# Critical-Infrastructure-Systems-Lab/ldsr

Hardware: AMD Instinct MI355X
Metric: restart x EM-iteration / s (T=1000, p=1, q=2) (higher is better)
Workload: dtype f64; 1 GPU; cfg2: synthetic T=1000 p=1 q=2, 1 series x 4096 restarts/GPU, niter=100, tol=0, dense mask; cells_rank0=4096, cells_total=4096, niter=100, algo=3

## Files before the change

include/ldsr_hip.h:

```cpp
#ifndef LDSR_HIP_H
#define LDSR_HIP_H

#include <stddef.h>

#ifdef __cplusplus
extern "C" {
#endif

#define LDSR_OK 0
#define LDSR_EINVAL 1
#define LDSR_EUNSUPPORTED 2
#define LDSR_EHIP 3
#define LDSR_EINTERRUPTED 4
#define LDSR_EINTERNAL 5

#define LDSR_CELL_OK 0
#define LDSR_CELL_NONFINITE 1
#define LDSR_CELL_SINGULAR 2
#define LDSR_CELL_INTERRUPTED 3

#define LDSR_ALGO_AUTO 0
#define LDSR_ALGO_SERIAL 1
#define LDSR_ALGO_SCAN 2
#define LDSR_ALGO_PAIR 3
// ... 29 lines not shown
int ldsr_em_restart_groups(int n_devices, const int *devices, int n_groups, ldsr_group *groups,
                           int niter, double tol, int algo);

int ldsr_em_batch(int device, int n_series, int T, int p, int q, const double *y,
                  const double *u, const double *v, int shared_uv, const int *cell_offsets,
                  const double *theta0, int niter, double tol, int algo,
                  double *theta, double *lik, int *n_iter, int *status, double *liks);

int ldsr_em_batch_multi(int n_devices, const int *devices, int n_series, int T, int p, int q,
                        const double *y, const double *u, const double *v, int shared_uv,
                        const int *cell_offsets, const double *theta0, int niter, double tol,
                        int algo, double *theta, double *lik, int *n_iter, int *status,
                        double *liks);

size_t ldsr_em_workspace_bytes(int n_series, int T, int p, int q, int n_cells, int algo);
int ldsr_em_batch_device(int device, void *stream, int n_series, int T, int p, int q,
                         const double *d_y, const double *d_u, const double *d_v,
                         int shared_uv, const int *cell_offsets, const double *d_theta0,
                         int niter, double tol, int algo, double *d_theta, double *d_lik,
                         int *d_n_iter, int *d_status, double *d_liks, void *d_workspace,
                         size_t workspace_bytes);

int ldsr_em_plan(int T, int p, int q, int niter, double tol, int algo, char *buf, size_t len);

int ldsr_em_batch_device_lead(int device, void *stream, int n_series, int T, int p, int q,
                              const double *d_y, const double *d_u, const double *d_v,
                              int shared_uv, const int *cell_offsets, const double *d_theta0,
                              int niter, double tol, int algo, double *d_theta, double *d_lik,
                              int *d_n_iter, int *d_status, double *d_liks, void *d_workspace,
                              size_t workspace_bytes, int lead_steps);
// ... 107 lines not shown
```

ldsr_amd/_lib.py:

```python
import ctypes as C
import os

_HERE = os.path.dirname(os.path.abspath(__file__))
SO_PATH = os.environ.get("LDSR_HIP_SO") or os.path.join(_HERE, "libldsr_hip.so")

_dp = C.POINTER(C.c_double)
_ip = C.POINTER(C.c_int)
_vp = C.c_void_p

SIGNATURES = {
    "ldsr_last_error": (C.c_char_p, []),
    "ldsr_version": (C.c_char_p, []),
    "ldsr_source_hash": (C.c_char_p, []),
    "ldsr_device_count": (C.c_int, []),
    "ldsr_shutdown": (None, []),
    "ldsr_em_batch": (C.c_int, [C.c_int, C.c_int, C.c_int, C.c_int, C.c_int, _dp, _dp, _dp,
                                C.c_int, _ip, _dp, C.c_int, C.c_double, C.c_int, _dp, _dp, _ip,
                                _ip, _dp]),
    "ldsr_em_batch_multi": (C.c_int, [C.c_int, _ip, C.c_int, C.c_int, C.c_int, C.c_int, _dp, _dp, _dp,
                                      C.c_int, _ip, _dp, C.c_int, C.c_double, C.c_int, _dp, _dp,
                                      _ip, _ip, _dp]),
    "ldsr_em_restart_grid": (C.c_int, [C.c_int, _ip, C.c_int, C.c_int, C.c_int, C.c_int, _dp, _dp, _dp,
                                       C.c_int, _ip, _dp, C.c_int, C.c_double, C.c_int, _dp, _dp,
                                       _ip, _ip, _ip, _dp, _dp, _ip, _dp, _dp, _dp, _dp, _dp]),
    "ldsr_em_restart_groups": (C.c_int, [C.c_int, _ip, C.c_int, _vp, C.c_int, C.c_double, C.c_int]),
    "ldsr_em_plan": (C.c_int, [C.c_int, C.c_int, C.c_int, C.c_int, C.c_double, C.c_int, C.c_char_p,
                               C.c_size_t]),
    "ldsr_em_plan_lead": (C.c_int, [C.c_int, C.c_int, C.c_int, C.c_int, C.c_double, C.c_int, C.c_int,
                                    C.c_char_p, C.c_size_t]),
    "ldsr_em_batch_device_lead": (C.c_int, [C.c_int, _vp, C.c_int, C.c_int, C.c_int, C.c_int, _vp, _vp,
                                            _vp, C.c_int, _ip, _vp, C.c_int, C.c_double, C.c_int, _vp,
                                            _vp, _vp, _vp, _vp, _vp, C.c_size_t, C.c_int]),
    "ldsr_smooth_plan": (C.c_int, [C.c_int, C.c_int, C.c_int, C.c_char_p, C.c_size_t]),
    "ldsr_kernel_inventory": (C.c_size_t, [C.c_char_p, C.c_size_t]),
    "ldsr_last_em_kernel": (C.c_int, [C.c_int, C.c_char_p, C.c_size_t]),
    "ldsr_set_interrupt_callback": (C.c_int, [_vp, _vp]),
    "ldsr_em_workspace_bytes": (C.c_size_t, [C.c_int, C.c_int, C.c_int, C.c_int, C.c_int, C.c_int]),
    "ldsr_em_batch_device": (C.c_int, [C.c_int, _vp, C.c_int, C.c_int, C.c_int, C.c_int, _vp, _vp,
                                       _vp, C.c_int, _ip, _vp, C.c_int, C.c_double, C.c_int, _vp,
                                       _vp, _vp, _vp, _vp, _vp, C.c_size_t]),
    "ldsr_smooth_batch": (C.c_int, [C.c_int, C.c_int, C.c_int, C.c_int, C.c_int, _dp, _dp, _dp,
                                    C.c_int, _ip, _dp, C.c_int, _dp, _dp, _dp, _dp, _dp]),
    "ldsr_mstep_batch": (C.c_int, [C.c_int, C.c_int, C.c_int, C.c_int, C.c_int, _dp, _dp, _dp,
                                   C.c_int, _ip, _dp, _dp, _dp, _dp, _ip]),
    "ldsr_propagate_batch": (C.c_int, [C.c_int, C.c_int, C.c_int, C.c_int, C.c_int, _dp, _dp, _dp,
                                       C.c_int, _ip, _dp, C.c_int, _dp, _dp, _dp, _dp]),
    "ldsr_penalized_lik_batch": (C.c_int, [C.c_int, C.c_int, C.c_int, C.c_int, C.c_int, _dp, _dp, _dp,
                                           C.c_int, _ip, _dp, C.c_double, _dp]),
    "ldsr_ga_batch": (C.c_int, [C.c_int, C.c_int, C.c_int, C.c_int, C.c_int, _dp, _dp, _dp, C.c_int, _dp, _dp,
                                C.c_double, C.c_int, C.c_int, C.c_int, C.c_int, C.c_ulonglong, _dp, C.c_int,
                                _dp, _dp, _ip, _dp, _dp, _dp]),
    "ldsr_ssq_grad_batch": (C.c_int, [C.c_int, C.c_int, C.c_int, C.c_int, C.c_int, _dp, _dp, _dp, C.c_int, _ip,
# ... 92 lines not shown
```

ldsr_amd/csrc/api_em.hip:

```cpp
#include <hip/hip_runtime.h>

#include <algorithm>
#include <cstdio>
#include <cstring>
#include <mutex>
#include <string>
#include <vector>

#include "host_em.h"
#include "em_pair_impl.h"

namespace ldsr_host {

static int device_cu_count(int device) {
    if (device < 0) return 256;
    static std::mutex mu;
    static std::vector<int> cache;
    std::lock_guard<std::mutex> lk(mu);
    if ((int)cache.size() <= device) cache.resize((size_t)device + 1, 0);
    if (!cache[(size_t)device]) {
        int n = 0;
        if (hipDeviceGetAttribute(&n, hipDeviceAttributeMultiprocessorCount, device) != hipSuccess || n <= 0) n = 256;
        cache[(size_t)device] = n;
    }
// ... 1 lines not shown
}

static std::mutex g_last_mu;
static std::vector<std::string> g_last_kernel;
static void remember_kernel(int device, const char *name) {
    std::lock_guard<std::mutex> lk(g_last_mu);
    if ((int)g_last_kernel.size() <= device) g_last_kernel.resize((size_t)device + 1);
    g_last_kernel[(size_t)device] = name;
}
extern "C" int ldsr_last_em_kernel(int device, char *buf, size_t len) {
    std::lock_guard<std::mutex> lk(g_last_mu);
    if (device < 0 || (int)g_last_kernel.size() <= device || g_last_kernel[(size_t)device].empty() || !buf || !len)
        return -1;
    snprintf(buf, len, "%s", g_last_kernel[(size_t)device].c_str());
    return 0;
}

WsLayout ws_layout(int n_series, int T, int PP, int QQ, int shared_uv, int n_cells,
                   int algo, int cpb) {
    WsLayout L;
    size_t o = 0;
    L.sc = o; o = align256(o + sizeof(SeriesConst) * (size_t)n_series);
    L.yp = o; o = align256(o + sizeof(double) * (size_t)n_series * T);
    L.yz = o; o = align256(o + sizeof(double) * (size_t)n_series * T);
    const size_t nuv = shared_uv ? 1 : (size_t)n_series;
    L.up = o; o = align256(o + sizeof(double) * nuv * T * PP);
    L.vp = o; o = align256(o + sizeof(double) * nuv * T * QQ);
    em_scan_layout(T, PP, QQ, &L.img_L, &L.img_NL, &L.img_stride);
    L.img = o; o = align256(o + sizeof(double) * (size_t)L.img_stride * n_series);
    L.img2_stride = 0; L.img3_stride = 0;
    if (PP <= 8 && QQ <= 8 && algo != LDSR_ALGO_SERIAL) {
        L.img2_stride = pair_image_doubles(PP <= 4 && QQ <= 4 ? 32 : 16, PP, QQ, 32);
        L.img3_stride = (long)(T + 32) * PP;
    }
    L.img2 = o; o = align256(o + sizeof(double) * (size_t)L.img2_stride * n_series);
    L.img3 = o; o = align256(o + sizeof(double) * (size_t)L.img3_stride * n_series);
    if (L.img_stride) cpb = std::min(cpb, em_scan_cells_per_block(T, PP, QQ));
    if (PP <= 8 && QQ <= 8 && algo != LDSR_ALGO_SERIAL) cpb = std::min(cpb, 4);
    L.max_blocks = n_cells / cpb + n_series + 1;
    L.blk = o; o = align256(o + sizeof(int) * (3 * (size_t)L.max_blocks + (size_t)n_series + 1));
    L.soc = o; o = align256(o + sizeof(int) * (size_t)(n_cells > 0 ? n_cells : 1));
    L.queue = o; o = align256(o + sizeof(int) * (size_t)n_series);
    const bool may_order = PP <= 4 && QQ <= 4 && algo != LDSR_ALGO_SERIAL;
    L.perm = o; o = align256(o + (may_order ? sizeof(int) * (size_t)(n_cells > 0 ? n_cells : 1) : 0));
    L.perm_key = o; o = align256(o + (may_order ? sizeof(int) * (size_t)(n_cells > 0 ? n_cells : 1) : 0));
    L.scratch_stride = ((long)n_cells + 63) / 64 * 64;
    L.scratch = o;
    if (algo == LDSR_ALGO_SERIAL) o = align256(o + sizeof(double) * 2 * (size_t)T * L.scratch_stride);
    L.total = o;
    return L;
}

extern "C" size_t ldsr_em_workspace_bytes(int n_series, int T, int p, int q, int n_cells,
                                          int algo) {
    if (n_series < 1 || n_cells < 0) return 0;
    EmPlanIn in;
    in.T = T; in.p = p; in.q = q; in.niter = 2; in.algo = algo;
    const EmPlan pl = em_plan(in);
    if (!pl.ok) return 0;
    return ws_layout(n_series, T, pl.PP, pl.QQ, 0, n_cells, pl.algo_layout, pl.layout_cpb).total;
}

extern "C" int ldsr_em_plan_lead(int T, int p, int q, int niter, double tol, int algo, int lead_steps,
                                 char *buf, size_t len) {
    EmPlanIn in;
    in.T = T; in.p = p; in.q = q; in.niter = niter; in.tol = tol; in.algo = algo; in.lead_steps = lead_steps;
    const EmPlan pl = em_plan(in);
    if (!pl.ok) return -1;
    if (buf && len) em_plan_kernel_name(pl, buf, len);
    return pl.algo;
}

extern "C" int ldsr_em_plan(int T, int p, int q, int niter, double tol, int algo, char *buf,
                            size_t len) {
    return ldsr_em_plan_lead(T, p, q, niter, tol, algo, 0, buf, len);
// ... 81 lines not shown
        pp.img2_stride = L.img2_stride;
        pp.L2 = pl.chunk;
        pp.NL2 = pl.lpc;
        pp.lead = pl.lead;
        pp.img3 = (pl.lead > 0 && L.img3_stride) ? (double *)(ws + L.img3) : nullptr;
        pp.img3_stride = L.img3_stride;
    }
    if (pl.steady_order) {
        tab.insert(tab.end(), cell_offsets, cell_offsets + n_series + 1);
        pp.perm = (int *)(ws + L.perm);
        pp.perm_key = (int *)(ws + L.perm_key);
        pp.cell_off = d_tab + 3 * n_blocks;
        pp.theta0 = E.theta0;
        pp.order_cpb = pl.queue ? 0 : cpb;
        pp.order_ntr = pl.chunk - 1;
    }
    rc = stage_h2d_async(E.device, E.stream, d_tab, tab.data(), sizeof(int) * tab.size());
    if (rc) return rc;
    HIPCHK(launch_series_prep(pp, n_series, E.stream));

    EmParams prm;
    prm.T = T; prm.p = p; prm.q = q; prm.has_u = E.u != nullptr; prm.has_v = E.v != nullptr;
    prm.niter = E.niter; prm.n_cells = n_cells; prm.tol = E.tol;
    prm.liks_nanfill = E.liks_nanfill;
    prm.abort = E.abort_flag;
    prm.yp = (const double *)(ws + L.yp);
    prm.yz = (const double *)(ws + L.yz);
    prm.up = (const double *)(ws + L.up);
    prm.vp = (const double *)(ws + L.vp);
    prm.u_stride = E.shared_uv ? 0 : (long)T * PP;
// ... 7 lines not shown
    prm.img3_stride = pp.img3_stride;
    prm.fitX = prm.fitY = prm.fitV = prm.fitJ = prm.pen = nullptr;
    prm.lambda = 0.0;
    prm.stdlik = 1;
    prm.sc = (const SeriesConst *)(ws + L.sc);
    prm.blk_series = d_tab;
    prm.blk_cell0 = d_tab + n_blocks;
    prm.blk_ncell = d_tab + 2 * n_blocks;
    prm.theta0 = E.theta0;
    prm.theta = E.theta; prm.lik = E.lik; prm.liks = E.liks;
    prm.n_iter = E.n_iter; prm.status = E.status;
    prm.queue = (int *)(ws + L.queue);
    prm.perm = pl.steady_order ? (const int *)(ws + L.perm) : nullptr;
    prm.scratch = (double *)(ws + L.scratch);
    prm.scratch_stride = L.scratch_stride;
    int slot;
    HIPCHK(prof_begin(E.device, E.stream, &slot));
    char nm[160];
    em_plan_kernel_name(pl, nm, sizeof(nm));
    remember_kernel(E.device, nm);
    if (pl.cpw)
        HIPCHK(launch_em_pair(prm, PP, QQ, pl.lpc, n_blocks, pl.queue, E.stream));
    else if (pl.algo == LDSR_ALGO_SCAN)
        HIPCHK(launch_em_scan(prm, PP, QQ, n_blocks, pl.queue, false, E.stream));
    else
        HIPCHK(launch_em_serial(prm, PP, QQ, n_blocks, E.stream));
    HIPCHK(prof_end(E.stream, slot));
    return LDSR_OK;
}

// ... 120 lines not shown
```

ldsr_amd/csrc/em_pair_impl.h:

```cpp
#pragma once
#include <type_traits>
#include "em_scan_impl.h"

__host__ __device__ constexpr long pair_image_doubles(int L, int PP, int QQ, int LPC = 32) {
    return img_doubles(L, LPC, PP, QQ);
}
__host__ __device__ constexpr long pair_strip_doubles(int L) { return (long)64 * (L - 1); }

__host__ __device__ constexpr long pair_tri_doubles(int PP, int QQ, int LPC = 32) {
    return (long)LPC * 2 * scan_pairs(PP, QQ);
}
#ifndef LDSR_STEADY
#define LDSR_STEADY 1
#endif
#ifndef LDSR_STEADY_PF
#define LDSR_STEADY_PF 4
#endif
#ifndef LDSR_STEADY_PF2
#define LDSR_STEADY_PF2 6
#endif
#ifndef LDSR_STEADY_REREAD_U
#define LDSR_STEADY_REREAD_U 1
#endif
#ifndef LDSR_LEAD_CLOSED_VAR
// ... 871 lines not shown
struct PairCarry {
    Theta<PP, QQ> th;
    double lik, lik1, lik2;
    int it, cell, wit;
    bool alive;
#ifdef LDSR_SCAN_TIMING
    unsigned long long tick_[10], last_, real0_;
#endif
};
#ifdef LDSR_SCAN_TIMING
#define PAIR_TICK_REFS auto &tick_ = cs.tick_; auto &last_ = cs.last_;
#else
#define PAIR_TICK_REFS
#endif

__device__ __forceinline__ int pair_cell_at(const PairEnv &E, int c0, int pos) { return E.perm ? E.perm[c0 + pos] : c0 + pos; }

__device__ __forceinline__ void pair_mark_interrupted(const PairEnv &E, int cell) {
    const int P = 6 + E.p + E.q;
    for (int k = 0; k < P; k++) E.theta[(long)cell * P + k] = NAN;
    if (E.liks && E.liks_nanfill)
        for (int i = 0; i < E.niter; i++) E.liks[(long)cell * E.niter + i] = NAN;
    E.n_iter[cell] = 0;
    E.lik[cell] = NAN;
    E.status[cell] = 3;
}

struct PairVarBlk { double Vp, sg, r0, K, Vu, AVu, J, Vp1; bool st; };
template <int L>
__device__ __forceinline__ PairVarBlk pair_var_block(double V1, double A, double C, double Q, double R, bool live,
// ... 167 lines not shown
            }
        }
    } else if (active) {
        mstep_update_white<PP, QQ>(cs.th, S, (SeriesConstK)E.sc, E.T);
    }
}

template <int PP, int QQ, bool QUEUE>
__device__ __forceinline__ bool pair_need_lik(const PairEnv &E, const PairCarry<PP, QQ> &cs, bool active) {
    if constexpr (QUEUE || LDSR_LIK_ON_DEMAND == 0) return true;
    else if constexpr (LDSR_LIK_ON_DEMAND == 2) return false;
    else return __any(E.tol > 0.0 || E.liks != nullptr || (active && cs.it + 1 >= E.niter) ||
                      (E.abort != nullptr && ((cs.wit + 1) & 63) == 0)) != 0;
}

template <int PP, int QQ, int L, bool QUEUE>
__device__ __attribute__((noinline)) PairCarry<PP, QQ> pair_steady_g_phase(PairEnv Ev, PairCarry<PP, QQ> cs, bool slow,
                                                                           int c0, int nc) {
    constexpr int LPC = 32;
    extern __shared__ __attribute__((aligned(16))) double smem[];
    PAIR_TICK_REFS
    auto ui = [](int x) { return __builtin_amdgcn_readfirstlane(x); };
    auto up = [&](auto *ptr) {
        const unsigned long long v = (unsigned long long)ptr;
        const unsigned lo = (unsigned)__builtin_amdgcn_readfirstlane((int)(unsigned)v);
        const unsigned hi = (unsigned)__builtin_amdgcn_readfirstlane((int)(unsigned)(v >> 32));
        return (decltype(ptr))(((unsigned long long)hi << 32) | lo);
    };
    PairEnv E;
    E.T = ui(Ev.T); E.p = ui(Ev.p); E.q = ui(Ev.q); E.has_u = ui(Ev.has_u); E.has_v = ui(Ev.has_v);
    E.niter = ui(Ev.niter); E.liks_nanfill = ui(Ev.liks_nanfill); E.n_obs = ui(Ev.n_obs);
    E.tol = uniform_d(Ev.tol);
    E.sc = up(Ev.sc); E.queue_s = up(Ev.queue_s); E.perm = up(Ev.perm); E.theta0 = up(Ev.theta0);
    E.theta = up(Ev.theta); E.lik = up(Ev.lik); E.liks = up(Ev.liks); E.n_iter = up(Ev.n_iter);
    E.status = up(Ev.status); E.abort = up(Ev.abort);
    c0 = ui(c0); nc = ui(nc);
    const int lane = threadIdx.x & 63, wave = threadIdx.x >> 6;
    const int vl = lane & 31, hbase = lane & 32;
    const int T = E.T;
    const int nl = (T + L - 1) / L, rp = T - nl * (L - 1);
    const bool shape_ok = rp >= 1 && nl > 1;
    const double *ys = smem;
    double *hs = smem + pair_image_doubles(L, PP, QQ, LPC) + (long)wave * pair_strip_doubles(L) + lane;
    do {
        SCAN_TICK(7)
        const bool need_lik = pair_need_lik<PP, QQ, QUEUE>(E, cs, slow);
        PairSweepOut<PP, QQ> o;
        pair_generic_sweeps<PP, QQ, L, LPC, true, !QUEUE>(o, cs.th, ys, hs, 0u, lane, nl, rp, cs.th.mu1, cs.th.V1, need_lik);
        SCAN_TICK(6)
        pair_steady_finish<PP, QQ, QUEUE>(E, cs, o, 0.0, 0.0, slow, lane, c0, nc, nl - 1, need_lik);
        const PairVarBlk vb = pair_var_block<L>(cs.th.V1, cs.th.A, cs.th.C, cs.th.Q, cs.th.R, cs.alive, vl, hbase, shape_ok);
        slow = cs.alive && !vb.st;
    } while (__any(slow));
    return cs;
}

template <int PP, int QQ, int L, bool QUEUE>
__device__ __forceinline__ void em_pair_body_steady(const EmParams &prm, const double *ys, double *hs,
                                                    const double *tri, int s, int c0, int nc, int lane,
                                                    int wave) {
    constexpr int LPC = 32;
    constexpr int KP = scan_pairs(PP, QQ), KV = img_values(PP, QQ);
    constexpr int NTR = L - 1;
    static_assert(NTR < LPC, "the last lane of the cell is the template, not a transient step");
    const int vl = lane & 31, hbase = lane & 32;
// ... 9 lines not shown
    const int P = 6 + prm.p + prm.q;
    PairEnv E;
    E.T = T; E.p = prm.p; E.q = prm.q; E.has_u = prm.has_u; E.has_v = prm.has_v;
    E.niter = prm.niter; E.liks_nanfill = prm.liks_nanfill; E.tol = prm.tol;
    E.sc = prm.sc + s; E.n_obs = E.sc->n_obs;
    E.queue_s = prm.queue + s; E.perm = prm.perm; E.theta0 = prm.theta0;
    E.theta = prm.theta; E.lik = prm.lik; E.liks = prm.liks; E.n_iter = prm.n_iter; E.status = prm.status;
    E.abort = prm.abort;
    const int nl = (T + L - 1) / L;
    const int rp = T - nl * (L - 1);
    const bool act = vl < nl;
    const bool tail = vl < rp;
    const int lastLane = nl - 1;
    const bool shape_ok = rp >= 1 && nl > 1;

    PairCarry<PP, QQ> cs;
    int k = QUEUE ? 0 : 2 * wave + (lane >> 5);
    if constexpr (QUEUE) {
        if (vl == 0) k = atomicAdd(E.queue_s, 1);
        k = __shfl(k, hbase, 64);
    }
    cs.alive = k < nc;
    cs.cell = pair_cell_at(E, c0, cs.alive ? k : 0);
    load_theta(cs.th, prm.theta0 + (long)cs.cell * P, prm.p, prm.q, prm.has_u, prm.has_v);
    white_in(cs.th, (SeriesConstK)E.sc);
    cs.lik = NAN; cs.lik1 = NAN; cs.lik2 = NAN;
    cs.it = 0;
    cs.wit = 0;
#ifdef LDSR_SCAN_TIMING
    for (int k_ = 0; k_ < 10; k_++) cs.tick_[k_] = 0;
    cs.last_ = __builtin_readcyclecounter();
    cs.real0_ = __builtin_amdgcn_s_memrealtime();
#endif
    PAIR_TICK_REFS
    Theta<PP, QQ> &th = cs.th;

    while (__any(cs.alive)) {
        bool slow = false;
        while (__any(cs.alive)) {
            SCAN_TICK(7)
            const double A = th.A, C = th.C;
            const PairVarBlk vb = pair_var_block<L>(th.V1, A, C, th.Q, th.R, cs.alive, vl, hbase, shape_ok);
            const bool st = vb.st;
            slow = cs.alive && !st;
            if (__builtin_expect(__any(slow), 0)) break;
            const bool need_lik = pair_need_lik<PP, QQ, QUEUE>(E, cs, cs.alive);
            double likq = 0.0, lsp = 0.0, tLv = 0.0, X0v = 0.0, V0v = 0.0;
            double addPall = 0.0, addTx1x = 0.0;
            double aSyx = 0.0, aTx1x = 0.0, aPall = 0.0;
            double aSxv[QQ], aTx1u[PP], aTux[PP];
            auto zero_sums = [&]() {
                aSyx = 0.0; aTx1x = 0.0; aPall = 0.0;
#pragma unroll
                for (int q_ = 0; q_ < QQ; q_++) aSxv[q_] = 0.0;
#pragma unroll
                for (int p_ = 0; p_ < PP; p_++) { aTx1u[p_] = 0.0; aTux[p_] = 0.0; }
            };
            const bool trl = vl < NTR;
            auto tval = [&](int i) -> double { return tri[((i >> 1) * LPC + vl) * 2 + (i & 1)]; };
            double e_t = tval(0), bu_t = 0.0;
// ... 273 lines not shown
                            const double ut = tval2(1 + p_);
                            aTx1u[p_] = fma(XsN, ut, aTx1u[p_]);
                            aTux[p_] = fma(ut, XsT, aTux[p_]);
                        }
                        aPall += fma(XsT, XsT, VsT);
                        aSyx = fma(tval2(0), XsT, aSyx);
#pragma unroll
                        for (int q_ = 0; q_ < QQ; q_++) aSxv[q_] = fma(XsT, tval2(1 + PP + q_), aSxv[q_]);
                    }
                    X0v = XsT; V0v = VsT;
                }
            } else {
                zero_sums();
            }
            SCAN_TICK(5)
            PairSweepOut<PP, QQ> o;
            o.aSyx = aSyx; o.aTx1x = aTx1x; o.aPall = aPall; o.aSxx = 0.0;
            o.likq = likq; o.lsp = lsp; o.tLv = tLv; o.X0v = X0v; o.V0v = V0v; o.sneg = 0;
#pragma unroll
            for (int q_ = 0; q_ < QQ; q_++) o.aSxv[q_] = aSxv[q_];
#pragma unroll
            for (int p_ = 0; p_ < PP; p_++) { o.aTx1u[p_] = aTx1u[p_]; o.aTux[p_] = aTux[p_]; }
            pair_steady_finish<PP, QQ, QUEUE>(E, cs, o, addTx1x, addPall, st, lane, c0, nc, lastLane, need_lik);
        }
        if (__builtin_expect(!__any(slow), 1)) break;
        cs = pair_steady_g_phase<PP, QQ, L, QUEUE>(E, cs, slow, c0, nc);
    }
}

template <int PP, int QQ, int L, int LPC, bool QUEUE, bool LEAD = false>
__global__ __launch_bounds__(512) void em_pair_kernel(EmParams prm) {
    extern __shared__ __attribute__((aligned(16))) double smem[];
    constexpr long IMG = pair_image_doubles(L, PP, QQ, LPC);
    const int b = blockIdx.x;
    const int s = prm.blk_series[b];
    const int c0 = prm.blk_cell0[b], nc = prm.blk_ncell[b];
    const int lane = threadIdx.x & 63, wave = threadIdx.x >> 6;
    const double *gimg = prm.img2 + (long)s * prm.img2_stride;
    for (int i = threadIdx.x; i < (int)IMG; i += blockDim.x) smem[i] = gimg[i];
    constexpr long STRIP = pair_strip_doubles(L);
    double *lu = smem + IMG + (long)(blockDim.x >> 6) * STRIP;
// ... 61 lines not shown
```

ldsr_amd/csrc/host_em.h:

```cpp
#pragma once
#include <vector>

#include "host_runtime.h"
#include "ldsr_kernels.h"

namespace ldsr_host {

struct WsLayout {
    size_t sc, yp, yz, up, vp, img, img2, img3, blk, soc, queue, perm, perm_key, scratch, total;
    long scratch_stride, img_stride;
    long img2_stride;
    long img3_stride;
    int max_blocks, img_L, img_NL;
};

WsLayout ws_layout(int n_series, int T, int PP, int QQ, int shared_uv, int n_cells, int algo, int cpb);
PrepParams prep_params(int n_series, int T, int p, int q, int PP, int QQ, const double *d_y, const double *d_u,
                       const double *d_v, int shared_uv, char *ws, const WsLayout &L, bool scan_img);

struct EmLaunch {
    int device = 0;
    hipStream_t stream = nullptr;
    int n_series = 0, T = 0, p = 0, q = 0, shared_uv = 0, niter = 0, algo = LDSR_ALGO_AUTO;
    double tol = 0.0;
// ... 58 lines not shown
```

ldsr_amd/csrc/kernels_serial.hip:

```cpp
#include "ldsr_device.h"
#include <cstdio>

#include "ldsr_kernels.h"

typedef volatile double *vdp;

__device__ static bool invert_small(double *a_, double *inv_, int n, int lane) {
    vdp a = a_, inv = inv_;
    constexpr int M = LDSR_MAXPQ;
    const int j = lane & 15, rg = lane >> 4;
    const bool col = j < n;
    for (int r = rg; r < n; r += 4)
        if (col) inv[r * M + j] = (r == j) ? 1.0 : 0.0;
    for (int c = 0; c < n; c++) {
        int piv = c;
        double best = fabs(a[c * M + c]);
        for (int r = c + 1; r < n; r++) {
            const double m = fabs(a[r * M + c]);
            if (m > best) { best = m; piv = r; }
        }
        if (!(best > 0.0) || !isfinite(best)) return false;
        if (piv != c && rg == 0 && col) {
            double t = a[c * M + j];
            a[c * M + j] = a[piv * M + j];
// ... 147 lines not shown
    const int T = prm.T, p = prm.p, q = prm.q, PP = prm.PP, QQ = prm.QQ;
    const int tid = threadIdx.x, lane = tid & 63, wave = tid >> 6;
    const int NT = blockDim.x, n_waves = NT >> 6;
    const double *y = prm.y + (long)s * T;
    const bool own_uv = (!prm.shared_uv) || s == 0;
    const double *u = prm.u ? prm.u + (prm.shared_uv ? 0 : (long)s * T * p) : nullptr;
    const double *v = prm.v ? prm.v + (prm.shared_uv ? 0 : (long)s * T * q) : nullptr;
    double *yp = prm.yp + (long)s * T;
    double *up = prm.up + (prm.shared_uv ? 0 : (long)s * T * PP);
    double *vp = prm.vp + (prm.shared_uv ? 0 : (long)s * T * QQ);

    __shared__ SeriesConst sc;
    __shared__ double inv_ws[LDSR_MAXPQ * LDSR_MAXPQ];

    if (tid == 0 && prm.queue) prm.queue[s] = 0;
    for (int t = tid; t < T; t += NT) {
        const double yv = y[t];
        yp[t] = yv;
        prm.yz[(long)s * T + t] = isfinite(yv) ? yv : 0.0;
    }
    if (own_uv) {
        for (int i = tid; i < T * PP; i += NT) {
            const int t = i / PP, k = i - t * PP;
            up[i] = (u && k < p && t < T - 1) ? u[(long)t * p + k] : 0.0;
        }
        for (int i = tid; i < T * QQ; i += NT) {
            const int t = i / QQ, k = i - t * QQ;
            vp[i] = (v && k < q) ? v[(long)t * q + k] : 0.0;
        }
    }
// ... 574 lines not shown
```

ldsr_amd/csrc/ldsr_device.h:

```cpp
#pragma once
#include <hip/hip_runtime.h>

#define LDSR_MAXPQ 16

struct SeriesConst {
    int n_obs;
    int status;
    int t_first_obs, t_last_obs;
    double Syy;
    double Syv[LDSR_MAXPQ];
    double wv[LDSR_MAXPQ];
    double Svv_inv[LDSR_MAXPQ * LDSR_MAXPQ];
    double Tuu_inv[LDSR_MAXPQ * LDSR_MAXPQ];
    double rn_obs, rTm1;
    double Lv[LDSR_MAXPQ * LDSR_MAXPQ], Lv_inv[LDSR_MAXPQ * LDSR_MAXPQ];
    double Lu[LDSR_MAXPQ * LDSR_MAXPQ], Lu_inv[LDSR_MAXPQ * LDSR_MAXPQ];
    double Syv_w[LDSR_MAXPQ];
};

template <int PP, int QQ>
struct Theta {
    double A, C, Q, R, mu1, V1;
    double B[PP], D[QQ];
};
// ... 230 lines not shown
    long img3_stride;
    const SeriesConst *sc;
    const int *blk_series, *blk_cell0, *blk_ncell;
    int *queue;
    const int *perm;
    const double *theta0;
    double *theta, *lik, *liks;
    int *n_iter, *status;
    const int *abort;
    double *scratch;
    long scratch_stride;
    double *fitX, *fitY, *fitV, *fitJ;
    double *pen;
    double lambda;
    int stdlik;
};

__device__ __forceinline__ int ldsr_poll_abort(const int *flag) {
    return __hip_atomic_load(flag, __ATOMIC_RELAXED, __HIP_MEMORY_SCOPE_SYSTEM);
}

__host__ __device__ constexpr int img_values(int PP, int QQ) { return 1 + PP + QQ; }
__host__ __device__ constexpr long img_doubles(int L, int NL, int PP, int QQ) {
    const int K = img_values(PP, QQ);
    return (long)NL * 2 * (L * (K / 2) + (K & 1) * ((L + 1) / 2));
}
__host__ __device__ constexpr int img_off(int j, int i, int K, int NL, int L) {
    const int KH = K / 2;
    return i < 2 * KH ? ((j * KH + (i >> 1)) * NL) * 2 + (i & 1)
                      : (L * KH + (j >> 1)) * NL * 2 + (j & 1);
// ... 4 lines not shown
```

ldsr_amd/csrc/ldsr_kernels.h:

```cpp
#pragma once
#include <hip/hip_runtime.h>

#include "ldsr_device.h"

struct PrepParams {
    int T, p, q, PP, QQ, shared_uv;
    const double *y, *u, *v;
    double *yp, *up, *vp;
    double *yz;
    double *img;
    long img_stride;
    int L, NL;
    double *img2;
    long img2_stride;
    int L2, NL2;
    int lead;
    double *img3;
    long img3_stride;
    SeriesConst *sc;
    int *queue;
    int *perm;
    int *perm_key;
    const int *cell_off;
    const double *theta0;
    int n_series;
    int order_cpb;
    int order_ntr;
};

struct SmoothParams {
    int T, p, q, has_u, has_v, n_cells, stdlik, mode;
    const double *yp, *up, *vp;
    long u_stride, v_stride;
    const SeriesConst *sc;
    const int *series_of_cell;
    const double *theta;
    double *X, *Y, *V, *J, *lik;
    double *theta_out;
    int *status;
    double *pen;
    double lambda;
    int scalar_only;
// ... 101 lines not shown
```

Baseline: 613.3 million restart*EM-iter/s.

## Add cross-wave mailbox swapping of stalled pair-EM cells to rebalance divergence

Adds a global mailbox that lets a wave whose two half-wave cells diverge (one slow, one steady) publish the steady cell's state so another wave, whose cells have fallen behind in iteration count, can take it over through a CAS handoff. The goal is less half-wave idling when the cells in a pair need different treatment, so lanes stay busy with matched work. It costs extra workspace, atomic polls of a ring of slots during the steady loop, record stores and loads, and more code complexity. It is on by default unless LDSR_PAIR_SWAP=0, and only applies to the non-queue steady-order pair path.

```diff
diff --git a/include/ldsr_hip.h b/include/ldsr_hip.h
--- a/include/ldsr_hip.h
+++ b/include/ldsr_hip.h
@@ -67,6 +67,8 @@
                         double *liks);
 
 size_t ldsr_em_workspace_bytes(int n_series, int T, int p, int q, int n_cells, int algo);
+int ldsr_em_swap_stats(int device, const void *d_workspace, int n_series, int T, int p, int q, int shared_uv,
+                       int n_cells, int algo, long long *swaps, int *not_empty);
 int ldsr_em_batch_device(int device, void *stream, int n_series, int T, int p, int q,
                          const double *d_y, const double *d_u, const double *d_v,
                          int shared_uv, const int *cell_offsets, const double *d_theta0,
diff --git a/ldsr_amd/_lib.py b/ldsr_amd/_lib.py
--- a/ldsr_amd/_lib.py
+++ b/ldsr_amd/_lib.py
@@ -36,6 +36,8 @@
     "ldsr_last_em_kernel": (C.c_int, [C.c_int, C.c_char_p, C.c_size_t]),
     "ldsr_set_interrupt_callback": (C.c_int, [_vp, _vp]),
     "ldsr_em_workspace_bytes": (C.c_size_t, [C.c_int, C.c_int, C.c_int, C.c_int, C.c_int, C.c_int]),
+    "ldsr_em_swap_stats": (C.c_int, [C.c_int, C.c_void_p, C.c_int, C.c_int, C.c_int, C.c_int, C.c_int, C.c_int, C.c_int,
+                                     C.POINTER(C.c_longlong), C.POINTER(C.c_int)]),
     "ldsr_em_batch_device": (C.c_int, [C.c_int, _vp, C.c_int, C.c_int, C.c_int, C.c_int, _vp, _vp,
                                        _vp, C.c_int, _ip, _vp, C.c_int, C.c_double, C.c_int, _vp,
                                        _vp, _vp, _vp, _vp, _vp, C.c_size_t]),
diff --git a/ldsr_amd/csrc/api_em.hip b/ldsr_amd/csrc/api_em.hip
--- a/ldsr_amd/csrc/api_em.hip
+++ b/ldsr_amd/csrc/api_em.hip
@@ -39,6 +39,11 @@
         return -1;
     snprintf(buf, len, "%s", g_last_kernel[(size_t)device].c_str());
     return 0;
+}
+
+static bool pair_swap_enabled() {
+    static const bool on = [] { const char *e = getenv("LDSR_PAIR_SWAP"); return !(e && e[0] == '0'); }();
+    return on;
 }
 
 WsLayout ws_layout(int n_series, int T, int PP, int QQ, int shared_uv, int n_cells,
@@ -69,6 +74,10 @@
     const bool may_order = PP <= 4 && QQ <= 4 && algo != LDSR_ALGO_SERIAL;
     L.perm = o; o = align256(o + (may_order ? sizeof(int) * (size_t)(n_cells > 0 ? n_cells : 1) : 0));
     L.perm_key = o; o = align256(o + (may_order ? sizeof(int) * (size_t)(n_cells > 0 ? n_cells : 1) : 0));
+    const bool may_swap = may_order && algo == LDSR_ALGO_PAIR;
+    L.mbox_slots = may_swap ? psw_total_slots(n_cells, n_series) : 0;
+    L.mbox = o; o = align256(o + (may_swap ? sizeof(psw_u64) * ((size_t)n_series + (size_t)L.mbox_slots) : 0));
+    L.mbox_rec = o; o = align256(o + sizeof(psw_u64) * (size_t)psw_rec_index(L.mbox_slots, 0));
     L.scratch_stride = ((long)n_cells + 63) / 64 * 64;
     L.scratch = o;
     if (algo == LDSR_ALGO_SERIAL) o = align256(o + sizeof(double) * 2 * (size_t)T * L.scratch_stride);
@@ -84,6 +93,25 @@
     const EmPlan pl = em_plan(in);
     if (!pl.ok) return 0;
     return ws_layout(n_series, T, pl.PP, pl.QQ, 0, n_cells, pl.algo_layout, pl.layout_cpb).total;
+}
+
+extern "C" int ldsr_em_swap_stats(int device, const void *d_workspace, int n_series, int T, int p, int q,
+                                  int shared_uv, int n_cells, int algo, long long *swaps, int *not_empty) {
+    if (n_series < 1 || n_cells < 0 || !d_workspace) return fail(LDSR_EINVAL, "bad swap-stats arguments");
+    EmPlanIn in;
+    in.T = T; in.p = p; in.q = q; in.niter = 2; in.algo = algo;
+    const EmPlan pl = em_plan(in);
+    if (!pl.ok) return fail(pl.err, pl.msg);
+    const WsLayout L = ws_layout(n_series, T, pl.PP, pl.QQ, shared_uv, n_cells, pl.algo_layout, pl.layout_cpb);
+    if (swaps) for (int s = 0; s < n_series; s++) swaps[s] = 0;
+    if (not_empty) *not_empty = 0;
+    if (!L.mbox_slots) return LDSR_OK;
+    HIPCHK(hipSetDevice(device));
+    std::vector<psw_u64> w((size_t)n_series + (size_t)L.mbox_slots);
+    HIPCHK(hipMemcpy(w.data(), (const char *)d_workspace + L.mbox, sizeof(psw_u64) * w.size(), hipMemcpyDeviceToHost));
+    if (swaps) for (int s = 0; s < n_series; s++) swaps[s] = (long long)w[(size_t)L.mbox_slots + (size_t)s];
+    if (not_empty) for (size_t i = 0; i < (size_t)L.mbox_slots; i++) *not_empty += w[i] != PSW_EMPTY;
+    return LDSR_OK;
 }
 
 extern "C" int ldsr_em_plan_lead(int T, int p, int q, int niter, double tol, int algo, int lead_steps,
@@ -195,6 +223,11 @@
         pp.theta0 = E.theta0;
         pp.order_cpb = pl.queue ? 0 : cpb;
         pp.order_ntr = pl.chunk - 1;
+    }
+    const bool swap = pair_swap_enabled() && pl.steady_order && !pl.queue && L.mbox_slots > 0 && n_cells > 2;
+    if (L.mbox_slots > 0) {
+        pp.mbox_zero = (psw_u64 *)(ws + L.mbox);
+        pp.mbox_zero_n = (long)n_series + L.mbox_slots;
     }
     rc = stage_h2d_async(E.device, E.stream, d_tab, tab.data(), sizeof(int) * tab.size());
     if (rc) return rc;
@@ -232,6 +265,10 @@
     prm.perm = pl.steady_order ? (const int *)(ws + L.perm) : nullptr;
     prm.scratch = (double *)(ws + L.scratch);
     prm.scratch_stride = L.scratch_stride;
+    prm.mbox_state = swap ? (psw_u64 *)(ws + L.mbox) : nullptr;
+    prm.mbox_cnt = swap ? (psw_u64 *)(ws + L.mbox) + L.mbox_slots : nullptr;
+    prm.mbox_rec = swap ? (psw_u64 *)(ws + L.mbox_rec) : nullptr;
+    prm.mbox_off = swap ? pp.cell_off : nullptr;
     int slot;
     HIPCHK(prof_begin(E.device, E.stream, &slot));
     char nm[160];
diff --git a/ldsr_amd/csrc/em_pair_impl.h b/ldsr_amd/csrc/em_pair_impl.h
--- a/ldsr_amd/csrc/em_pair_impl.h
+++ b/ldsr_amd/csrc/em_pair_impl.h
@@ -1,6 +1,7 @@
 #pragma once
 #include <type_traits>
 #include "em_scan_impl.h"
+#include "pair_swap.h"
 
 __host__ __device__ constexpr long pair_image_doubles(int L, int PP, int QQ, int LPC = 32) {
     return img_doubles(L, LPC, PP, QQ);
@@ -909,6 +910,22 @@
 #define PAIR_TICK_REFS
 #endif
 
+template <int PP, int QQ>
+struct PairCarrySwap : PairCarry<PP, QQ> {
+    psw_u64 *cnt_s, *state, *rec;
+    int lo, n, me;
+    int pj;
+    unsigned sw;
+};
+__device__ __forceinline__ constexpr int pair_sw_tries(unsigned sw) { return (int)(sw & 15u); }
+__device__ __forceinline__ constexpr int pair_sw_taken(unsigned sw) { return (int)((sw >> 4) & 15u); }
+__device__ __forceinline__ constexpr unsigned pair_sw_seq(unsigned sw) { return sw >> 8; }
+__device__ __forceinline__ constexpr unsigned pair_sw_pack(int tries, int taken, unsigned seq) {
+    return (unsigned)tries | ((unsigned)taken << 4) | (seq << 8);
+}
+template <int PP, int QQ, bool QUEUE>
+using PairCarryOf = std::conditional_t<QUEUE, PairCarry<PP, QQ>, PairCarrySwap<PP, QQ>>;
+
 __device__ __forceinline__ int pair_cell_at(const PairEnv &E, int c0, int pos) { return E.perm ? E.perm[c0 + pos] : c0 + pos; }
 
 __device__ __forceinline__ void pair_mark_interrupted(const PairEnv &E, int cell) {
@@ -1106,9 +1123,88 @@
                       (E.abort != nullptr && ((cs.wit + 1) & 63) == 0)) != 0;
 }
 
+template <int PP, int QQ>
+__device__ __forceinline__ psw_u64 pair_rec_word(const PairCarry<PP, QQ> &cs, int k) {
+    double w = cs.th.A;
+    auto put = [&](int i, double v) { w = k == i ? v : w; };
+    put(1, cs.th.C); put(2, cs.th.Q); put(3, cs.th.R); put(4, cs.th.mu1); put(5, cs.th.V1);
+#pragma unroll
+    for (int p_ = 0; p_ < PP; p_++) put(6 + p_, cs.th.B[p_]);
+#pragma unroll
+    for (int q_ = 0; q_ < QQ; q_++) put(6 + PP + q_, cs.th.D[q_]);
+    put(6 + PP + QQ, cs.lik); put(7 + PP + QQ, cs.lik1); put(8 + PP + QQ, cs.lik2);
+    const psw_u64 tail = ((psw_u64)(unsigned)cs.it << 32) | (psw_u64)(unsigned)cs.cell;
+    return k == 9 + PP + QQ ? tail : (psw_u64)__double_as_longlong(w);
+}
+template <int PP, int QQ>
+constexpr int pair_rec_words() { return 10 + PP + QQ; }
+template <int PP, int QQ>
+__device__ __forceinline__ void pair_rec_adopt(PairCarry<PP, QQ> &cs, psw_u64 x, bool mine) {
+    static_assert(pair_rec_words<PP, QQ>() <= PSW_REC_WORDS, "a record is one 256-byte line");
+    const double xd = __longlong_as_double((long long)x);
+    auto set = [&](double &f, int i) { const double v = readlane_d(xd, i); f = mine ? v : f; };
+    set(cs.th.A, 0); set(cs.th.C, 1); set(cs.th.Q, 2); set(cs.th.R, 3); set(cs.th.mu1, 4); set(cs.th.V1, 5);
+#pragma unroll
+    for (int p_ = 0; p_ < PP; p_++) set(cs.th.B[p_], 6 + p_);
+#pragma unroll
+    for (int q_ = 0; q_ < QQ; q_++) set(cs.th.D[q_], 6 + PP + q_);
+    set(cs.lik, 6 + PP + QQ); set(cs.lik1, 7 + PP + QQ); set(cs.lik2, 8 + PP + QQ);
+    const psw_u64 tail = (psw_u64)__double_as_longlong(readlane_d(xd, 9 + PP + QQ));
+    if (mine) { cs.it = (int)(unsigned)(tail >> 32); cs.cell = (int)(unsigned)tail; cs.alive = true; }
+}
+__device__ __forceinline__ psw_u64 pair_uniform_u64(psw_u64 v) {
+    const unsigned lo = (unsigned)__builtin_amdgcn_readfirstlane((int)(unsigned)v);
+    const unsigned hi = (unsigned)__builtin_amdgcn_readfirstlane((int)(unsigned)(v >> 32));
+    return ((psw_u64)hi << 32) | lo;
+}
+template <int PP, int QQ>
+__device__ __forceinline__ void pair_swap_uniform(PairCarrySwap<PP, QQ> &cs) {
+    auto ui = [](int x) { return __builtin_amdgcn_readfirstlane(x); };
+    cs.cnt_s = (psw_u64 *)pair_uniform_u64((psw_u64)cs.cnt_s);
+    cs.state = (psw_u64 *)pair_uniform_u64((psw_u64)cs.state);
+    cs.rec = (psw_u64 *)pair_uniform_u64((psw_u64)cs.rec);
+    cs.lo = ui(cs.lo); cs.n = ui(cs.n); cs.me = ui(cs.me); cs.pj = ui(cs.pj); cs.sw = (unsigned)ui((int)cs.sw);
+}
+template <int PP, int QQ>
+__device__ __forceinline__ bool pair_swap_wanted(const PairCarry<PP, QQ> &cs, int seen_it) {
+    return __any(psw_behind(seen_it, cs.it)) != 0;
+}
+template <int PP, int QQ>
+__device__ __forceinline__ void pair_swap_take(PairCarrySwap<PP, QQ> &cs, int lane) {
+    constexpr int NW = pair_rec_words<PP, QQ>();
+    const int vl = lane & 31, hbase = lane & 32;
+    if (!cs.state) return;
+    int tries = pair_sw_tries(cs.sw) - 1, nsw = pair_sw_taken(cs.sw);
+    cs.sw = pair_sw_pack(tries, nsw, pair_sw_seq(cs.sw));
+    psw_u64 *st = cs.state + cs.pj;
+    psw_u64 seen = 0;
+    if (lane == 0) seen = PSW_LOAD(st);
+    seen = pair_uniform_u64(seen);
+    const unsigned long long am = __ballot(cs.alive);
+    const int it0 = __builtin_amdgcn_readlane(cs.it, 0), it1 = __builtin_amdgcn_readlane(cs.it, 32);
+    const int adv = it1 > it0 ? 32 : 0;
+    const bool both = (am & 1ull) != 0ull && ((am >> 32) & 1ull) != 0ull;
+    const bool mine = cs.pj >= cs.lo && cs.pj < cs.lo + cs.n;
+    if (!mine || !both || nsw >= PSW_MAX_SWAPS || !psw_wants(seen, max(it0, it1))) return;
+    PSW_ACQUIRE();
+    psw_u64 x = 0;
+    if (vl < NW) x = PSW_LOAD(cs.rec + psw_rec_index(cs.pj, 0) + vl);
+    const psw_u64 w = pair_rec_word<PP, QQ>(cs, vl);
+    if (hbase == adv && vl < NW) PSW_STORE(cs.rec + psw_rec_index(cs.me, 1 + nsw) + vl, w);
+    PSW_DRAIN();
+    int won = 0;
+    if (lane == 0) won = psw_take(st, seen, cs.me, nsw) ? 1 : 0;
+    won = __builtin_amdgcn_readfirstlane(won);
+    if (!won) return;
+    pair_rec_adopt<PP, QQ>(cs, x, hbase == adv);
+    nsw++;
+    cs.sw = pair_sw_pack(nsw >= PSW_MAX_SWAPS ? 0 : tries, nsw, pair_sw_seq(cs.sw));
+    if (lane == 0) PSW_ADD(cs.cnt_s, 1ull);
+}
+
 template <int PP, int QQ, int L, bool QUEUE>
-__device__ __attribute__((noinline)) PairCarry<PP, QQ> pair_steady_g_phase(PairEnv Ev, PairCarry<PP, QQ> cs, bool slow,
-                                                                           int c0, int nc) {
+__device__ __attribute__((noinline)) PairCarryOf<PP, QQ, QUEUE> pair_steady_g_phase(PairEnv Ev, PairCarryOf<PP, QQ, QUEUE> cs,
+                                                                                    bool slow, int c0, int nc) {
     constexpr int LPC = 32;
     extern __shared__ __attribute__((aligned(16))) double smem[];
     PAIR_TICK_REFS
@@ -1129,6 +1225,13 @@
     c0 = ui(c0); nc = ui(nc);
     const int lane = threadIdx.x & 63, wave = threadIdx.x >> 6;
     const int vl = lane & 31, hbase = lane & 32;
+    if constexpr (!QUEUE) {
+        pair_swap_uniform<PP, QQ>(cs);
+        if (!__any(slow)) {
+            pair_swap_take<PP, QQ>(cs, lane);
+            return cs;
+        }
+    }
     const int T = E.T;
     const int nl = (T + L - 1) / L, rp = T - nl * (L - 1);
     const bool shape_ok = rp >= 1 && nl > 1;
@@ -1136,11 +1239,52 @@
     double *hs = smem + pair_image_doubles(L, PP, QQ, LPC) + (long)wave * pair_strip_doubles(L) + lane;
     do {
         SCAN_TICK(7)
+        psw_u64 offer = PSW_EMPTY;
+        int ph = 0;
+        if constexpr (!QUEUE) {
+            if (cs.state) {
+                const unsigned long long sm = __ballot(slow), am = __ballot(cs.alive);
+                const bool s0 = (sm & 1ull) != 0ull, s1 = ((sm >> 32) & 1ull) != 0ull;
+                const bool both = (am & 1ull) != 0ull && ((am >> 32) & 1ull) != 0ull;
+                const bool polls = E.abort != nullptr && ((cs.wit + 1) & 63) == 0;
+                if (both && s0 != s1 && !polls) {
+                    constexpr int NW = pair_rec_words<PP, QQ>();
+                    ph = s0 ? 32 : 0;
+                    int vk = vl;
+                    asm volatile("" : "+v"(vk));
+                    const psw_u64 w = pair_rec_word<PP, QQ>(cs, vl);
+                    if (hbase == ph && vl < NW) PSW_STORE(cs.rec + psw_rec_index(cs.me, 0) + vk, w);
+                    cs.sw += 1u << 8;
+                    offer = psw_offer_word(pair_sw_seq(cs.sw), __builtin_amdgcn_readlane(cs.it, ph));
+                    PSW_DRAIN();
+                    if (lane == 0) psw_publish(cs.state + cs.me, offer);
+                    if (hbase == ph) cs.alive = false;
+                }
+            }
+        }
         const bool need_lik = pair_need_lik<PP, QQ, QUEUE>(E, cs, slow);
         PairSweepOut<PP, QQ> o;
         pair_generic_sweeps<PP, QQ, L, LPC, true, !QUEUE>(o, cs.th, ys, hs, 0u, lane, nl, rp, cs.th.mu1, cs.th.V1, need_lik);
         SCAN_TICK(6)
         pair_steady_finish<PP, QQ, QUEUE>(E, cs, o, 0.0, 0.0, slow, lane, c0, nc, nl - 1, need_lik);
+        if constexpr (!QUEUE) {
+            if (offer != PSW_EMPTY) {
+                psw_u64 r = PSW_EMPTY;
+                if (lane == 0) r = psw_resolve(cs.state + cs.me, offer);
+                r = pair_uniform_u64(r);
+                if (hbase == ph) cs.alive = true;
+                if (r != PSW_EMPTY) {
+                    constexpr int NW = pair_rec_words<PP, QQ>();
+                    PSW_ACQUIRE();
+                    psw_u64 x = 0;
+                    int vk = vl;
+                    asm volatile("" : "+v"(vk));
+                    if (vl < NW) x = PSW_LOAD(cs.rec + psw_rec_index(psw_taken_slot(r), 1 + psw_taken_give(r)) + vk);
+                    pair_rec_adopt<PP, QQ>(cs, x, hbase == ph);
+                    if (lane == 0) psw_clear(cs.state + cs.me);
+                }
+            }
+        }
         const PairVarBlk vb = pair_var_block<L>(cs.th.V1, cs.th.A, cs.th.C, cs.th.Q, cs.th.R, cs.alive, vl, hbase, shape_ok);
         slow = cs.alive && !vb.st;
     } while (__any(slow));
@@ -1180,11 +1324,31 @@
     const int lastLane = nl - 1;
     const bool shape_ok = rp >= 1 && nl > 1;
 
-    PairCarry<PP, QQ> cs;
+    PairCarryOf<PP, QQ, QUEUE> cs;
     int k = QUEUE ? 0 : 2 * wave + (lane >> 5);
     if constexpr (QUEUE) {
         if (vl == 0) k = atomicAdd(E.queue_s, 1);
         k = __shfl(k, hbase, 64);
+    }
+    psw_u64 *pp = nullptr;
+    int seen_it = PSW_NO_IT, swap_args = 0;
+    if constexpr (!QUEUE) {
+        cs.cnt_s = nullptr; cs.state = nullptr; cs.rec = nullptr; cs.lo = 0; cs.n = 0; cs.me = 0; cs.pj = 0;
+        cs.sw = pair_sw_pack(PSW_MAX_TRIES, 0, 0u);
+        if (prm.mbox_state) {
+            const int off_s = prm.mbox_off[s];
+            const int lo = psw_slot_base(off_s, s), n = psw_slot_count(prm.mbox_off[s + 1] - off_s);
+            const int me = lo + ((c0 - off_s) >> 1) + wave;
+            if (n > 1) {
+                pp = prm.mbox_state + me;
+                auto put = [&](int k_, unsigned v) { swap_args = lane == k_ ? (int)v : swap_args; };
+                auto put2 = [&](int k_, const void *ptr) {
+                    put(k_, (unsigned)(unsigned long long)ptr); put(k_ + 1, (unsigned)((unsigned long long)ptr >> 32));
+                };
+                put2(0, prm.mbox_cnt + s); put2(2, prm.mbox_state); put2(4, prm.mbox_rec);
+                put(6, (unsigned)lo); put(7, (unsigned)n); put(8, (unsigned)me);
+            }
+        }
     }
     cs.alive = k < nc;
     cs.cell = pair_cell_at(E, c0, cs.alive ? k : 0);
@@ -1202,14 +1366,15 @@
     Theta<PP, QQ> &th = cs.th;
 
     while (__any(cs.alive)) {
-        bool slow = false;
+        bool slow = false, swp = false;
         while (__any(cs.alive)) {
             SCAN_TICK(7)
             const double A = th.A, C = th.C;
             const PairVarBlk vb = pair_var_block<L>(th.V1, A, C, th.Q, th.R, cs.alive, vl, hbase, shape_ok);
             const bool st = vb.st;
             slow = cs.alive && !st;
-            if (__builtin_expect(__any(slow), 0)) break;
+            if constexpr (!QUEUE) swp = pair_swap_wanted<PP, QQ>(cs, seen_it);
+            if (__builtin_expect(__any(slow) || swp, 0)) break;
             const bool need_lik = pair_need_lik<PP, QQ, QUEUE>(E, cs, cs.alive);
             double likq = 0.0, lsp = 0.0, tLv = 0.0, X0v = 0.0, V0v = 0.0;
             double addPall = 0.0, addTx1x = 0.0;
@@ -1513,6 +1678,13 @@
                 zero_sums();
             }
             SCAN_TICK(5)
+            if constexpr (!QUEUE) {
+                if (__builtin_amdgcn_readfirstlane((int)((unsigned long long)pp >> 32)) != 0) {
+                    constexpr unsigned long long RB = PSW_RING * sizeof(psw_u64) - 1;
+                    pp = (psw_u64 *)(((unsigned long long)pp & ~RB) | (((unsigned long long)pp + sizeof(psw_u64)) & RB));
+                    seen_it = psw_it(PSW_LOAD(pp));
+                }
+            }
             PairSweepOut<PP, QQ> o;
             o.aSyx = aSyx; o.aTx1x = aTx1x; o.aPall = aPall; o.aSxx = 0.0;
             o.likq = likq; o.lsp = lsp; o.tLv = tLv; o.X0v = X0v; o.V0v = V0v; o.sneg = 0;
@@ -1522,8 +1694,19 @@
             for (int p_ = 0; p_ < PP; p_++) { o.aTx1u[p_] = aTx1u[p_]; o.aTux[p_] = aTux[p_]; }
             pair_steady_finish<PP, QQ, QUEUE>(E, cs, o, addTx1x, addPall, st, lane, c0, nc, lastLane, need_lik);
         }
-        if (__builtin_expect(!__any(slow), 1)) break;
+        if (__builtin_expect(!__any(slow) && !swp, 1)) break;
+        if constexpr (!QUEUE) {
+            auto get = [&](int k_) { return (unsigned)__builtin_amdgcn_readlane(swap_args, k_); };
+            auto get2 = [&](int k_) { return (psw_u64 *)(((unsigned long long)get(k_ + 1) << 32) | get(k_)); };
+            cs.cnt_s = get2(0); cs.state = get2(2); cs.rec = get2(4);
+            cs.lo = (int)get(6); cs.n = (int)get(7); cs.me = (int)get(8);
+            cs.pj = pp ? (int)(pp - cs.state) : cs.me;
+        }
         cs = pair_steady_g_phase<PP, QQ, L, QUEUE>(E, cs, slow, c0, nc);
+        if constexpr (!QUEUE) {
+            if (pair_sw_tries(cs.sw) <= 0) pp = nullptr;
+            seen_it = PSW_NO_IT;
+        }
     }
 }
 
diff --git a/ldsr_amd/csrc/host_em.h b/ldsr_amd/csrc/host_em.h
--- a/ldsr_amd/csrc/host_em.h
+++ b/ldsr_amd/csrc/host_em.h
@@ -7,7 +7,8 @@
 namespace ldsr_host {
 
 struct WsLayout {
-    size_t sc, yp, yz, up, vp, img, img2, img3, blk, soc, queue, perm, perm_key, scratch, total;
+    size_t sc, yp, yz, up, vp, img, img2, img3, blk, soc, queue, perm, perm_key, mbox, mbox_rec, scratch, total;
+    long mbox_slots;
     long scratch_stride, img_stride;
     long img2_stride;
     long img3_stride;
diff --git a/ldsr_amd/csrc/kernels_serial.hip b/ldsr_amd/csrc/kernels_serial.hip
--- a/ldsr_amd/csrc/kernels_serial.hip
+++ b/ldsr_amd/csrc/kernels_serial.hip
@@ -1,6 +1,7 @@
 #include "ldsr_device.h"
 #include <cstdio>
 
+#include "pair_swap.h"
 #include "ldsr_kernels.h"
 
 typedef volatile double *vdp;
@@ -185,6 +186,9 @@
     __shared__ double inv_ws[LDSR_MAXPQ * LDSR_MAXPQ];
 
     if (tid == 0 && prm.queue) prm.queue[s] = 0;
+    if (prm.mbox_zero)
+        for (long i = (long)s * NT + tid; i < prm.mbox_zero_n; i += (long)prm.n_series * NT)
+            prm.mbox_zero[i] = i < prm.mbox_zero_n - prm.n_series ? PSW_EMPTY : 0ull;
     for (int t = tid; t < T; t += NT) {
         const double yv = y[t];
         yp[t] = yv;
diff --git a/ldsr_amd/csrc/ldsr_device.h b/ldsr_amd/csrc/ldsr_device.h
--- a/ldsr_amd/csrc/ldsr_device.h
+++ b/ldsr_amd/csrc/ldsr_device.h
@@ -268,6 +268,10 @@
     double *pen;
     double lambda;
     int stdlik;
+    unsigned long long *mbox_state;
+    unsigned long long *mbox_cnt;
+    unsigned long long *mbox_rec;
+    const int *mbox_off;
 };
 
 __device__ __forceinline__ int ldsr_poll_abort(const int *flag) {
diff --git a/ldsr_amd/csrc/ldsr_kernels.h b/ldsr_amd/csrc/ldsr_kernels.h
--- a/ldsr_amd/csrc/ldsr_kernels.h
+++ b/ldsr_amd/csrc/ldsr_kernels.h
@@ -26,6 +26,8 @@
     int n_series;
     int order_cpb;
     int order_ntr;
+    unsigned long long *mbox_zero;
+    long mbox_zero_n;
 };
 
 struct SmoothParams {
diff --git a/ldsr_amd/csrc/pair_swap.h b/ldsr_amd/csrc/pair_swap.h
--- /dev/null
+++ b/ldsr_amd/csrc/pair_swap.h
@@ -0,0 +1,69 @@
+#pragma once
+
+#if defined(__HIPCC__)
+#define PSW_HD __host__ __device__
+#define PSW_FN __host__ __device__ __forceinline__
+#else
+#define PSW_HD
+#define PSW_FN inline
+#endif
+#if defined(__HIP_DEVICE_COMPILE__)
+#define PSW_G(p) ((__attribute__((address_space(1))) unsigned long long *)(unsigned long long)(p))
+#define PSW_LOAD(p) __hip_atomic_load(PSW_G(p), __ATOMIC_RELAXED, __HIP_MEMORY_SCOPE_AGENT)
+#define PSW_STORE(p, v) __hip_atomic_store(PSW_G(p), (v), __ATOMIC_RELAXED, __HIP_MEMORY_SCOPE_AGENT)
+#define PSW_CAS(p, e, d) __hip_atomic_compare_exchange_strong(PSW_G(p), (e), (d), __ATOMIC_RELAXED, __ATOMIC_RELAXED, __HIP_MEMORY_SCOPE_AGENT)
+#define PSW_ADD(p, v) __hip_atomic_fetch_add(PSW_G(p), (v), __ATOMIC_RELAXED, __HIP_MEMORY_SCOPE_AGENT)
+#define PSW_DRAIN() asm volatile("s_waitcnt vmcnt(0)" ::: "memory")
+#define PSW_ACQUIRE() __builtin_amdgcn_fence(__ATOMIC_ACQUIRE, "agent")
+#else
+#define PSW_LOAD(p) __atomic_load_n((p), __ATOMIC_ACQUIRE)
+#define PSW_STORE(p, v) __atomic_store_n((p), (v), __ATOMIC_RELEASE)
+#define PSW_CAS(p, e, d) __atomic_compare_exchange_n((p), (e), (d), false, __ATOMIC_ACQ_REL, __ATOMIC_ACQUIRE)
+#define PSW_ADD(p, v) __atomic_fetch_add((p), (v), __ATOMIC_RELAXED)
+#define PSW_DRAIN() ((void)0)
+#define PSW_ACQUIRE() ((void)0)
+#endif
+
+typedef unsigned long long psw_u64;
+
+constexpr int PSW_REC_WORDS = 32;
+constexpr int PSW_RECS = 3;
+constexpr int PSW_MAX_SWAPS = 2;
+constexpr int PSW_MAX_TRIES = 4;
+constexpr int PSW_RING = 32;
+PSW_HD constexpr long psw_total_slots(long n_cells, long n_series) {
+    return (n_cells / 2 + n_series + 1 + PSW_RING - 1) / PSW_RING * PSW_RING;
+}
+PSW_HD constexpr long psw_next_slot(long slot) { return (slot & ~(long)(PSW_RING - 1)) | ((slot + 1) & (PSW_RING - 1)); }
+PSW_HD constexpr int psw_slot_base(int off_s, int s) { return (off_s >> 1) + s; }
+PSW_HD constexpr int psw_slot_count(int n_s) { return (n_s + 1) >> 1; }
+PSW_HD constexpr long psw_rec_index(long slot, int rec) { return (slot * PSW_RECS + rec) * PSW_REC_WORDS; }
+
+constexpr unsigned PSW_K_EMPTY = 0u, PSW_K_OFFER = 1u, PSW_K_TAKEN = 2u;
+constexpr int PSW_NO_IT = 0x7fffffff;
+constexpr psw_u64 PSW_EMPTY = (psw_u64)(unsigned)PSW_NO_IT << 32;
+PSW_HD constexpr unsigned psw_kind(psw_u64 w) { return (unsigned)(w & 3ull); }
+PSW_HD constexpr int psw_it(psw_u64 w) { return (int)(unsigned)(w >> 32); }
+PSW_HD constexpr psw_u64 psw_offer_word(unsigned seq, int it) {
+    return (psw_u64)PSW_K_OFFER | ((psw_u64)(seq & 0x3fffffffu) << 2) | ((psw_u64)(unsigned)it << 32);
+}
+PSW_HD constexpr psw_u64 psw_taken_word(int slot, int give) {
+    return PSW_EMPTY | (psw_u64)PSW_K_TAKEN | ((psw_u64)(unsigned)give << 2) | ((psw_u64)(unsigned)slot << 4);
+}
+PSW_HD constexpr int psw_taken_slot(psw_u64 w) { return (int)((unsigned)w >> 4); }
+PSW_HD constexpr int psw_taken_give(psw_u64 w) { return (int)((w >> 2) & 3ull); }
+PSW_HD constexpr bool psw_behind(int seen_it, int it_adv) { return seen_it < it_adv; }
+PSW_HD constexpr bool psw_wants(psw_u64 seen, int it_adv) {
+    return psw_kind(seen) == PSW_K_OFFER && psw_behind(psw_it(seen), it_adv);
+}
+
+PSW_FN void psw_publish(psw_u64 *state, psw_u64 offer) { PSW_STORE(state, offer); }
+PSW_FN psw_u64 psw_resolve(psw_u64 *state, psw_u64 offer) {
+    psw_u64 e = offer;
+    return PSW_CAS(state, &e, PSW_EMPTY) ? PSW_EMPTY : e;
+}
+PSW_FN void psw_clear(psw_u64 *state) { PSW_STORE(state, PSW_EMPTY); }
+PSW_FN bool psw_take(psw_u64 *state, psw_u64 seen, int own_slot, int give) {
+    psw_u64 e = seen;
+    return PSW_CAS(state, &e, psw_taken_word(own_slot, give));
+}
```

Measured after the change: 628.8 million restart*EM-iter/s (median of 6 runs). 2.5% higher.
